# devitocodes/seigen

Hardware: AMD Instinct MI355X
Metric: M DoF-updates/sec, 3D elastic P=4 (higher is better)
Workload: dtype f64

## Files before the change

### seigen_amd/csrc/api.cpp

```cpp
#include <limits>
#include <string>

#include "handle.hpp"
#include "source_tables.hpp"
#include "sponge_tables.hpp"

static int init_element(const sg_config* cfg, sg_handle* h) {
  if (cfg->dim < 1 || cfg->dim > 3) return fail(h, SG_ERR_ARG, "dim must be 1, 2 or 3");
  if (cfg->degree < 1 || cfg->degree > 4) return fail(h, SG_ERR_ARG, "degree must be 1..4");
  for (int a = 0; a < cfg->dim; ++a) {
    if (cfg->n[a] < 1) return fail(h, SG_ERR_ARG, "n[axis] must be >= 1");
    if (!(cfg->h[a] > 0.0)) return fail(h, SG_ERR_ARG, "h[axis] must be > 0");
  }
  h->cfg = *cfg;
  for (int a = cfg->dim; a < 3; ++a) {
    h->cfg.n[a] = 1;
    h->cfg.h[a] = 1.0;
    h->cfg.origin[a] = 0.0;
    h->cfg.cube0[a] = 0;
  }
  int ndev = 0;
  if (hipGetDeviceCount(&ndev) != hipSuccess || ndev <= 0)
    return fail(h, SG_ERR_DEVICE, "no HIP device available (libseigen_hip has no CPU fallback)");
  if (cfg->device < 0 || cfg->device >= ndev) return fail(h, SG_ERR_ARG, "device ordinal out of range");
// ... 97 lines not shown
      Dt = hexm_table(cfg->degree, Dt.data(), Dt.data() + (size_t)(cfg->degree + 1) * (cfg->degree + 1), h->md);
      break;
    }
    case Family::Lane: {
      if (hex) break;
      double fact = 1.0;
      for (int i = 2; i <= d - 1; ++i) fact *= i;
      const double cfold = 1.0 / (2.0 * fact);
      for (int r = 0; r < d; ++r)
        for (int a = 0; a < nd; ++a)
          for (int b = 0; b < nd; ++b) {
            double v = re.D[((size_t)r * nd + a) * nd + b];
            for (int bf = 0; bf < nf; ++bf) {
              if (re.fnode[(size_t)0 * nf + bf] == b) v -= cfold * re.L[((size_t)0 * nd + a) * nf + bf];
              if (re.fnode[(size_t)(r + 1) * nf + bf] == b) v += cfold * re.L[((size_t)(r + 1) * nd + a) * nf + bf];
            }
            Dt[((size_t)r * nd + a) * nd + b] = v;
          }
      Lt = re.L;
      break;
    }
    case Family::Mfma: {
      if (h->f32) set_frags(fr, mfma32_frags_F(re), mfma32_frags_G(re), mfma32_frags_L(re));
      else set_frags(fr, mfma_frags_F(re), mfma_frags_G(re), mfma_frags_L(re));
      const char* gq = std::getenv("SEIGEN_HIP_GQ");
      if (!h->f32 && cfg->degree >= 3 && (gq ? std::atoi(gq) != 0 : cfg->degree >= SG_GQ_FROM_DEGREE)) {
        try {
          fr[3] = mfma_frags_Q(re);
          fr[4] = mfma_frags_P(re);
        } catch (const std::exception& e) {
          return fail(h, SG_ERR_ARG, e.what());
        }
      }
      break;
    }
    case Family::Tile2d: {
      h->t2c = tile2d_const(h->md);
      if (h->f32) set_frags(fr, tile2d_frags32_V(re, -1.0), tile2d_frags32_V(re, 1.0), tile2d_frags32_L(re));
      else set_frags(fr, tile2d_frags_V(re, -1.0), tile2d_frags_V(re, 1.0), tile2d_frags_L(re));
      break;
    }
  }
  HIPCHECK(h, h->Dt.upload(Dt.data(), Dt.size()));
  HIPCHECK(h, h->Lt.upload(Lt.data(), Lt.size()));
  HIPCHECK(h, h->md_dev.upload(&h->md, 1));
  if (h->family == Family::Mfma) {
    const MfmaConst mk = mfma_const(h->md);
    HIPCHECK(h, h->mk_dev.upload(&mk, 1));
    std::vector<int32_t> ft, tab;
    mfma_trace_offsets(h->md, 9, ft);
    HIPCHECK(h, h->ftab_dev.upload(ft.data(), ft.size()));
    if ((h->md.ncube_pad / 16) * 6 * 16 >= ((int64_t)1 << 31))
      return fail(h, SG_ERR_ARG, "block too large for the MFMA path's neighbour table");
    build_nbr_table(h->md, tab);
    HIPCHECK(h, h->nbr_tab.upload(tab.data(), tab.size()));
  }
  return SG_OK;
}

static int init_fields(sg_handle* h, const Frags& fr) {
  const int d = h->cfg.dim, nd = h->re.nd;
  for (int f = 0; f < 4; ++f) {
    size_t comps = field_is_stress(f) ? (size_t)d * d : (size_t)d;
    h->field_len[f] = (size_t)h->ncells * nd * comps;
    h->field_alloc[f] = (size_t)h->md.ncube_pad * h->ncls * nd * comps;
    const size_t n = h->f32 ? (h->field_alloc[f] + 1) / 2 : h->field_alloc[f];
// ... 2 lines not shown
  }
  DevBuf<double>* frag[5] = {&h->fragF, &h->fragG, &h->fragL, &h->fragQ, &h->fragP};
  for (int i = 0; i < 5; ++i)
    if (!fr[i].empty()) HIPCHECK(h, frag[i]->upload(fr[i].data(), fr[i].size()));
  if (family_interleaved(h->family)) {
    const char* sym_env = std::getenv("SEIGEN_HIP_SYM");
    h->sym = !(sym_env && std::strcmp(sym_env, "0") == 0);
    const int zero = 0;
    HIPCHECK(h, h->sym_flag.upload(&zero, 1));
  }
  if (std::getenv("SEIGEN_HIP_STAMPS")) {
    const std::vector<unsigned long long> zeros(32, 0);
    HIPCHECK(h, h->dbg.upload(zeros.data(), zeros.size()));
  }
  return SG_OK;
}

static int blocks_per_cu(const sg_handle* h) {
  const int P = h->cfg.degree;
  return h->family == Family::Mfma ? mfma_blocks_per_cu(P, h->f32) : (h->family == Family::Hexm ? hexm_blocks_per_cu(P) : 2);
}

static int init_launch(sg_handle* h) {
  const sg_config* cfg = &h->cfg;
  hipDeviceProp_t prop;
  HIPCHECK(h, hipGetDeviceProperties(&prop, cfg->device));
  h->ncu = prop.multiProcessorCount;
  const int slots = blocks_per_cu(h) * prop.multiProcessorCount;
  h->grid_full = slots / 8 * 8;
  h->grid_blocks = (cfg->nbr_mask != 0 ? slots - slots / 16 : slots) / 8 * 8;
  if (const char* gb = std::getenv("SEIGEN_HIP_GRID_BLOCKS")) h->grid_blocks = std::max(8, std::atoi(gb) / 8 * 8);
  if (cfg->nbr_mask == 0) h->grid_full = h->grid_blocks;
  h->order_chunk = 0;
  if (h->family == Family::Mfma) {
    const int64_t per_layer = ((int64_t)cfg->n[0] * cfg->n[1] + 15) / 16 * 6;
    if (cfg->n[2] >= 16) h->order_chunk = (int)std::max<int64_t>(6, (per_layer + 7) / 8);
  }
  if (const char* oc = std::getenv("SEIGEN_HIP_ORDER_CHUNK")) h->order_chunk = std::max(0, std::atoi(oc));
  h->no_whole = std::getenv("SEIGEN_HIP_NO_WHOLE") != nullptr;
  h->tile_grid = 0;
  h->tile_grid_sponge = 2008;
  if (const char* tg = std::getenv("SEIGEN_HIP_TILE_GRID")) h->tile_grid = h->tile_grid_sponge = std::max(8, std::atoi(tg) / 8 * 8);
  const char* ge = std::getenv("SEIGEN_HIP_GRAPH");
  const int64_t dofs = h->ncells * (int64_t)h->re.nd * (cfg->dim + cfg->dim * cfg->dim);
  h->graph_ok = ge ? (std::strcmp(ge, "0") != 0) : (dofs <= (int64_t)1 << 23);
  const char* ov = std::getenv("SEIGEN_HIP_OVERLAP");
  h->overlap = cfg->nbr_mask != 0 && !(ov && std::strcmp(ov, "0") == 0);
  int prio_lo = 0, prio_hi = 0;
  HIPCHECK(h, hipDeviceGetStreamPriorityRange(&prio_lo, &prio_hi));
  if (cfg->stream) {
    h->stream = (hipStream_t)cfg->stream;
  } else {
    HIPCHECK(h, hipStreamCreateWithPriority(&h->stream, hipStreamNonBlocking, h->overlap ? prio_hi : 0));
    h->own_stream = true;
  }
  if (h->overlap) {
    HIPCHECK(h, hipStreamCreateWithPriority(&h->stream2, hipStreamNonBlocking, prio_lo));
    HIPCHECK(h, hipEventCreateWithFlags(&h->ev_stage, hipEventDisableTiming));
    HIPCHECK(h, hipEventCreateWithFlags(&h->ev_second, hipEventDisableTiming));
  }
  HIPCHECK(h, hipEventCreate(&h->ev0));
  HIPCHECK(h, hipEventCreate(&h->ev1));
  HIPCHECK(h, hipDeviceSynchronize());
  return SG_OK;
}

// ... 457 lines not shown
```

### seigen_amd/csrc/handle.hpp

```cpp
#pragma once
#include <hip/hip_runtime.h>

#include <cmath>
#include <algorithm>
#include <cstdio>
#include <cstdlib>
#include <cstring>
#include <string>
#include <thread>
#include <vector>

#include "../../include/seigen_hip.h"
#include "hostlogic.hpp"
#include "kernels.hpp"
#include "mesh_tables.hpp"
#include "mfma_tables.hpp"
#include "refelem.hpp"

using namespace sg;

struct sg_comm_state;

template <typename T>
struct DevBuf {
// ... 95 lines not shown
  const double* read(int f) const { return buf_[f].get(); }
  double* write(int f) {
    ver_.written(f);
    return buf_[f].get();
  }
  void replayed() { ver_.replayed(); }
  const FieldVersions& versions() const { return ver_; }
  hipError_t alloc(int f, size_t n) { return buf_[f].alloc(n); }

 private:
  DevBuf<double> buf_[4];
  FieldVersions ver_;
};

struct sg_handle {
  sg_config cfg;
  sg_comm_state* comm = nullptr;
  RefElem re;
  MeshDev md;
  DevBuf<MeshDev> md_dev;
  DevBuf<double> Dt, Lt;
  Fields field;
  size_t field_len[4] = {0, 0, 0, 0};
  size_t field_alloc[4] = {0, 0, 0, 0};
  Family family = Family::Generic;
  int f32 = 0;
  bool sym = false;
  DevBuf<int> sym_flag;
  DevBuf<int32_t> region_items[5];
  int32_t region_nitems[5] = {-1, -1, -1, -1, -1};
  bool region_whole[5] = {false, false, false, false, false};
  DevBuf<double> fragF, fragG, fragL;
  DevBuf<double> fragQ, fragP;
  DevBuf<double> staging;
  double* pin[2] = {nullptr, nullptr};
  DevBuf<double> dstage[2];
  hipEvent_t xfer_ev[2] = {nullptr, nullptr};
  DevBuf<unsigned long long> dbg;
  size_t staging_len = 0;
  int64_t ncells = 0;
  int ncls = 0;
  bool params_set = false;
  double rho = 1.0, dt = 0.0, lam0 = 0.0, mu0 = 0.0;
  int per_cell = 0;
  DevBuf<double> lam_d, mu_d;
  DevBuf<double> rho2_d;
  int rho_physical = 0;
  SpongeTables sponge;
  SourceTables src;
  int64_t src_step = 0;
  DevBuf<int64_t> src_ctr_d;
  bool graph_src = false;
  ReceiverTables rec;
  bool graph_rec = false;
  MonitorTables mon;
  MeasureScratch msr;
  bool graph_mon = false;
  const double* ghost[4][6] = {};
  hipStream_t stream = nullptr;
  bool own_stream = false;
  bool overlap = false;
  hipStream_t stream2 = nullptr;
  hipEvent_t ev_stage = nullptr, ev_second = nullptr;
  bool second_pending = false;
  DevBuf<int32_t> nbr_tab;
  DevBuf<MfmaConst> mk_dev;
// ... 71 lines not shown
```

### seigen_amd/csrc/kernels.hpp

```cpp
#pragma once
#include <cstdint>
#include <string>
#include <type_traits>
#include <vector>

#include "../../include/seigen_hip.h"
#include "mesh_tables.hpp"

namespace sg {

constexpr int SG_MAX_BOXES = 7;

template <int DIM, int P, int TP = 0>
struct ElemDims {
  static constexpr int ND = TP ? (DIM == 3 ? (P + 1) * (P + 1) * (P + 1) : (P + 1) * (P + 1))
                               : (DIM == 1) ? (P + 1) : (DIM == 2) ? (P + 1) * (P + 2) / 2 : (P + 1) * (P + 2) * (P + 3) / 6;
  static constexpr int NF = (DIM == 1) ? 1 : (DIM == 2) ? (P + 1) : (TP ? (P + 1) * (P + 1) : (P + 1) * (P + 2) / 2);
  static constexpr int NFACES = TP ? 2 * DIM : DIM + 1;
  static constexpr int NCLS = TP ? 1 : (DIM == 1) ? 1 : (DIM == 2) ? 2 : 6;
};

constexpr int MK_KSF = 4;
constexpr int MK_KS = 9;
#ifndef SG_GQ_FROM_DEGREE
// ... 50 lines not shown
  const double* Lt;
  const MeshDev* md;
  const MfmaConst* mk;
  const int32_t* ftab;
  const int32_t* nbr_tab;
  int32_t all_active;
  int32_t tensor;
  const double* fragV;
  const double* fragL;
  const double* fragQ;
  unsigned long long* dbg;
  const int32_t* sponge_slot;
  const double* sponge_B;
  const double* sponge_sigma;
  const void* sponge_pre;
  const double* lam;
  const double* mu;
  double lam0, mu0;
  double c_self, c_aux, c_new;
  const double* rho2;
  int32_t mode;
  int32_t per_cell;
  int32_t box_o[3], box_n[3];
  int32_t nbox;
  int32_t boxes_o[SG_MAX_BOXES][3], boxes_n[SG_MAX_BOXES][3];
  int32_t spread;
  const int32_t* item_list;
  int32_t nlist;
  int32_t sym;
  int32_t grid_blocks;
  int32_t f32;
  int32_t order_chunk;
  int32_t nitems;
  void* reserved_;
  const int32_t* src_slot;
  const int32_t* src_idx;
  const double* src_vals;
  double src_scale;
  double src_coef;
  SrcStep src_step;
  int32_t src_bump;
};

std::string kernel_name_of(const void* host_fn);

template <int V0, int... Vs, typename F>
auto sg_pick(int v, F&& f) {
  decltype(f(std::integral_constant<int, V0>())) r{};
  auto take = [&](auto c) { return v == c.value && ((r = f(c)), true); };
  (void)(take(std::integral_constant<int, V0>()) || ... || take(std::integral_constant<int, Vs>()));
  return r;
}
inline int any_ghost(const StageArgs& a, int nsides) {
  int g = 0;
  for (int sd = 0; sd < nsides; ++sd) g |= a.ghost[sd] != nullptr;
  return g;
}

const void* stage_kernel_generic(int kind, int dim, int P, const StageArgs& a);
int launch_stage(const void* kernel, int dim, int P, const StageArgs& a, void* stream);

int mfma_blocks_per_cu(int P, int f32);
const void* stage_kernel_mfma(int kind, int P, const StageArgs& a);
int launch_stage_mfma(const void* kernel, const StageArgs& a, void* stream);

const void* stage_kernel_lane(int kind, int dim, int P, const StageArgs& a);
int launch_stage_lane(const void* kernel, const StageArgs& a, long nitems, void* stream);
int hexm_blocks_per_cu(int P);
std::vector<double> hexm_table(int P, const double* D1, const double* lift1, const MeshDev& md_host);
const void* stage_kernel_hexm(int kind, int P, const StageArgs& a);
int launch_stage_hexm(const void* kernel, int P, const StageArgs& a, long nitems, void* stream);

struct T2Class {
  double Jinv[2][2], cn[4][2];
  int32_t nb_axis[4], nb_dir[4], nb_cls[4];
  int32_t slot_ord[4];
  uint32_t tfw[4][2];
  uint32_t tgw[4][2];
};
struct T2Const {
  int32_t n0, n1, ncube, ngroups;
  int32_t has_nbr[4];
  int32_t halo_per_cube;
  int32_t gpr;
  double inv_n0;
  uint32_t tpw[4][2];
  T2Class cls[2];
};
T2Const tile2d_const(const MeshDev& md_host);
const void* stage_kernel_tile2d(int kind, int P, const StageArgs& a);
int launch_stage_tile2d(const void* kernel, int resident, const StageArgs& a, const T2Const& c, long nitems, void* stream);

int launch_layout(const MeshDev& md_host, int ncomp, int dir, void* field, double* staging, int64_t cell0,
                  int64_t ncells, int sym, int* flag, int f32, void* stream);
int launch_mirror(const MeshDev& md_host, void* field, int f32, void* stream);
// ... 59 lines not shown
```

### seigen_amd/csrc/kernels_mfma.hip

```cpp
#include <hip/hip_runtime.h>

#include "kernels.hpp"

namespace sg {

template <typename R>
struct RT;
template <>
struct RT<double> {
  typedef double v4 __attribute__((ext_vector_type(4)));
  static constexpr bool SMALL = true;
  static __device__ __forceinline__ v4 big(double a, double b, v4 c) { return __builtin_amdgcn_mfma_f64_16x16x4f64(a, b, c, 0, 0, 0); }
  static __device__ __forceinline__ double small(double a, double b, double c) { return __builtin_amdgcn_mfma_f64_4x4x4f64(a, b, c, 0, 0, 0); }
};
template <>
struct RT<float> {
  typedef float v4 __attribute__((ext_vector_type(4)));
  static constexpr bool SMALL = false;
  static __device__ __forceinline__ v4 big(float a, float b, v4 c) { return __builtin_amdgcn_mfma_f32_16x16x4f32(a, b, c, 0, 0, 0); }
  static __device__ __forceinline__ float small(float, float, float c) { return c; }
};

template <typename R, int P>
constexpr int mfma_resident_blocks() {
  return sizeof(R) == 4 ? 3 : (P == 1 ? 4 : (P == 2 ? 3 : 2));
}

template <int P, typename R>
struct MG {
  static constexpr int ND = ElemDims<3, P>::ND;
  static constexpr int NF = ElemDims<3, P>::NF;
  static constexpr int KS = (ND + 3) / 4;
  static constexpr int KSF = (NF + 3) / 4;
  static constexpr int MTF = RT<R>::SMALL ? ND / 16 : (ND + 15) / 16;
  static constexpr int NSM = RT<R>::SMALL ? (ND % 16 + 3) / 4 : 0;
  static constexpr int MTT = MTF + NSM;
  static constexpr int MTFA = MTF > 0 ? MTF : 1;
  static constexpr int NSMA = NSM > 0 ? NSM : 1;
  static constexpr int S4 = (ND + 3) / 4;
  static constexpr int NFRAG_F = MTT * 3 * KS;
  static constexpr int NFRAG_G = 3 * MTT * KS;
  static constexpr int NFRAG_L = 4 * MTT * KSF;
  static constexpr int RK = (P >= 2) ? ElemDims<3, (P >= 2 ? P - 1 : 1)>::ND : 1;
  static constexpr int QLT = RK / 16;
  static constexpr int QST = (RK % 16 + 3) / 4;
  static constexpr int KR = (RK + 3) / 4;
  static constexpr int NFRAG_Q = (QLT + QST) * KS;
  static constexpr int NFRAG_P = 3 * MTT * KR;
};

#define LD_STREAM(p) __builtin_nontemporal_load(p)
#define ST_STREAM(p, v) __builtin_nontemporal_store((v), (p))
#define SG_PRIO(p) __builtin_amdgcn_s_setprio(p)
constexpr int SG_PRIO_F0 = 0x120, SG_PRIO_F1 = 0x320, SG_PRIO_F2 = 0x320, SG_PRIO_G0 = 0x120, SG_PRIO_G1 = 0x120;
#define SG_PRIO_VOL ((PRIO3 >> 8) & 3)
#define SG_PRIO_LIFT ((PRIO3 >> 4) & 3)
#define SG_PRIO_EPI (PRIO3 & 3)
#define MFMA64(a, b, c) RT<R>::big((a), (b), (c))
#define MFMA4(a, b, c) RT<R>::small((a), (b), (c))

#ifdef SG_STAMPS
#define STAMP(t)                                                                   \
  do {                                                                             \
    __builtin_amdgcn_sched_barrier(0);                                             \
    asm volatile("s_memtime %0\n\ts_waitcnt lgkmcnt(0)" : "=s"(t)::"memory");       \
    __builtin_amdgcn_sched_barrier(0);                                             \
  } while (0)
#define STAMP_DECL unsigned long long st0 = 0, st1 = 0, st2 = 0, st3 = 0, st4 = 0, sta = 0, stb = 0, sacc[4] = {0, 0, 0, 0}, ssub[3] = {0, 0, 0}, sitems = 0
#define STAMP_ACC                                                                  \
  do {                                                                             \
    sacc[0] += st1 - st0;                                                          \
    sacc[1] += st2 - st1;                                                          \
    sacc[2] += st3 - st2;                                                          \
    sacc[3] += st4 - st3;                                                          \
    if (sta) { ssub[0] += sta - st2; ssub[1] += stb - sta; ssub[2] += st3 - stb; } \
    sitems += 1;                                                                   \
  } while (0)
#define STAMP_FLUSH                                                                \
  do {                                                                             \
    if (A.dbg && lane == 0) {                                                      \
      for (int z = 0; z < 4; ++z) atomicAdd(&A.dbg[z], sacc[z]);                   \
// ... 162 lines not shown
    r.xcd = xcd;
    r.lo = slot * wpb + wave;
    r.hi = mine > 0 ? mine * chunk : 0;
    return r;
  }
  const long ipx = (nitems + 7) / 8;
  r.lo = xcd * ipx + slot * wpb + wave;
  r.hi = (xcd + 1) * ipx < nitems ? (xcd + 1) * ipx : nitems;
  return r;
}
__device__ __forceinline__ long item_of(const ItemRange& r, long it) {
  if (r.chunk == 0) return it;
  const long c = it / r.chunk;
  const long item = (c * 8 + r.xcd) * r.chunk + (it - c * r.chunk);
  return item < r.nitems ? item : -1;
}

template <int N, typename R, int NT = 256>
__device__ __forceinline__ void copy_to_lds(R* dst, const R* __restrict__ src) {
  constexpr int PER = (N + NT - 1) / NT;
  R v[PER];
#pragma unroll
  for (int j = 0; j < PER; ++j) {
    const int i = threadIdx.x + j * NT;
    v[j] = (i < N) ? src[i] : R(0);
  }
#pragma unroll
  for (int j = 0; j < PER; ++j) {
    const int i = threadIdx.x + j * NT;
    if (i < N) dst[i] = v[j];
  }
}

template <int NV, int NL, typename R, int NT = 256>
__device__ __forceinline__ void load_tables(R* sAV, R* sAL, const StageArgs& A) {
  copy_to_lds<NV * 64, R, NT>(sAV, reinterpret_cast<const R*>(A.fragV));
  copy_to_lds<NL * 64, R, NT>(sAL, reinterpret_cast<const R*>(A.fragL));
  __syncthreads();
}

template <int NV, int NL, typename R>
__device__ __forceinline__ void load_tables(R* sAV, R* sAL, MeshDev* sMd, const StageArgs& A) {
  const int* src = reinterpret_cast<const int*>(A.md);
  int* dst = reinterpret_cast<int*>(sMd);
  constexpr int NI = (int)(sizeof(MeshDev) / sizeof(int)), PERI = (NI + 255) / 256;
  int w[PERI];
#pragma unroll
  for (int j = 0; j < PERI; ++j) {
    const int i = threadIdx.x + j * 256;
    w[j] = (i < NI) ? src[i] : 0;
  }
  copy_to_lds<NV * 64>(sAV, reinterpret_cast<const R*>(A.fragV));
  copy_to_lds<NL * 64>(sAL, reinterpret_cast<const R*>(A.fragL));
#pragma unroll
  for (int j = 0; j < PERI; ++j) {
    const int i = threadIdx.x + j * 256;
    if (i < NI) dst[i] = w[j];
  }
  __syncthreads();
}


template <typename R>
__device__ __forceinline__ R ndot(R c0, R c1, R c2, R t0, R t1, R t2) {
  R r = c0 * t0;
  r = __builtin_fma(c1, t1, r);
  r = __builtin_fma(c2, t2, r);
  return r;
}
template <>
__device__ __forceinline__ float ndot<float>(float c0, float c1, float c2, float t0, float t1, float t2) {
  float r = c0 * t0;
  r = __builtin_fmaf(c1, t1, r);
  r = __builtin_fmaf(c2, t2, r);
  return r;
}


template <typename R, int P, int MODE, int SYM, int FACT>
__global__ __launch_bounds__(256, (mfma_resident_blocks<R, P>())) void mfma_stage_G(StageArgs A) {
  using M = MG<P, R>;
  typedef typename RT<R>::v4 d4;
  constexpr int PRIO3 = MODE ? SG_PRIO_G1 : SG_PRIO_G0;
  constexpr int ND = M::ND, NF = M::NF, KS = M::KS, KSF = M::KSF, MTF = M::MTF, NSM = M::NSM, MTT = M::MTT, S4 = M::S4;
  constexpr int PF = sizeof(R) == 4 ? 6 : 4;
  constexpr int QLT = M::QLT, QST = M::QST, KR = M::KR;
  __shared__ R sAV[(FACT ? M::NFRAG_P : M::NFRAG_G) * 64];
  __shared__ R sQ[FACT ? M::NFRAG_Q * 64 : 1];
  __shared__ R sAL[M::NFRAG_L * 64];
  __shared__ MeshDev sMd;
  if constexpr (FACT) copy_to_lds<M::NFRAG_Q * 64>(sQ, reinterpret_cast<const R*>(A.fragQ));
  load_tables<(FACT ? M::NFRAG_P : M::NFRAG_G), M::NFRAG_L>(sAV, sAL, &sMd, A);

  const int lane = threadIdx.x & 63;
  const int wave = __builtin_amdgcn_readfirstlane(threadIdx.x >> 6);
  const int q = lane >> 4, w = lane & 15;
  typedef __attribute__((address_space(4))) const MeshDev cMeshDev;
  const cMeshDev* md = (const cMeshDev*)(unsigned long long)A.md;
  const R* __restrict__ in = reinterpret_cast<const R*>(A.in);
  R* __restrict__ out = reinterpret_cast<R*>(A.out);
  const R c_self = (R)A.c_self, c_new = (R)A.c_new;
  const long ngroups = sMd.ncube_pad >> 4;
  const ItemRange ir = item_range(A.item_list ? (long)A.nlist : ngroups * 6, wave, A.spread, A.order_chunk);

  STAMP_DECL;
  for (long it = ir.lo; it < ir.hi; it += ir.step) {
    STAMP(st0);
    const long iti = item_of(ir, it);
    if (iti < 0) continue;
    const long item = A.item_list ? (long)A.item_list[iti] : iti;
    const long g = item / 6;
    const int k = (int)(item - g * 6);
    const LaneGeo L = A.all_active ? lane_geo_all(sMd.ncube, g, w) : lane_geo(sMd, A, g, w);
    const nbr4 nbe = load_nbr4(A, item, w);
    if (!__any(L.active)) continue;
    const R* own = in + ((g * 6 + k) * (long)ND) * 3 * 16 + w;
    int qo = q * 3 * 16;
    asm volatile("" : "+v"(qo));
    const R* ownq = own + qo;
    const R* ownl = (4 * (KS - 1) + q < ND) ? ownq + (KS - 1) * 4 * 3 * 16 : own;
    auto brow = [&](int ks) { return (ks == KS - 1) ? ownl : ownq + ks * 4 * 3 * 16; };
    int lo = lane;
    asm volatile("" : "+v"(lo));

    R Jm[3][3], cnf[4][3];
#pragma unroll
    for (int r = 0; r < 3; ++r)
#pragma unroll
      for (int j = 0; j < 3; ++j) Jm[r][j] = (R)(-md->Jinv[k][r][j]);
#pragma unroll
    for (int f = 0; f < 4; ++f)
#pragma unroll
      for (int j = 0; j < 3; ++j) cnf[f][j] = (R)md->cn[k][f][j];

    R Sd[3][S4], So[3][S4];
#pragma unroll
    for (int i = 0; i < 3; ++i)
#pragma unroll
      for (int m = 0; m < S4; ++m) Sd[i][m] = So[i][m] = R(0);

    constexpr int NB = 2;
    constexpr int NBO = FACT ? NB : 1;
    R nx[NB][KSF][3], nxo[NBO][KSF][3];
    auto request = [&](int f, R (&dst)[KSF][3], R (&dso)[KSF][3]) {
      const NbrRef<R> NR = nbr_from_entry<ND, NF, 3>(A, nbe[f], 2 * sMd.nb_axis[k][f] + (sMd.nb_dir[k][f] > 0 ? 1 : 0), own);
#pragma unroll
      for (int ks = 0; ks < KSF; ++ks) {
        const int bb = (4 * ks + q < NF) ? 4 * ks + q : 0;
        const int on = sMd.fnode[f][bb];
        const int nn = NR.ghost ? sMd.nb_fnode[k][f][bb] : (NR.physical ? on : sMd.nb_node[k][f][bb]);
#pragma unroll
        for (int i = 0; i < 3; ++i) {
          dst[ks][i] = NR.p[(nn * 3 + i) * NR.cstride];
          if constexpr (FACT) dso[ks][i] = own[(on * 3 + i) * 16];
        }
      }
    };
    SG_PRIO(SG_PRIO_VOL);
    STAMP(st1);
    auto fold_dir = [&](int r, const d4 (&acc)[M::MTFA][3], const R (&accs)[M::NSMA][3]) {
#pragma unroll
      for (int kk = 0; kk < 3; ++kk) {
        const R c = Jm[r][kk];
        if (uniform_nonzero(c)) {
#pragma unroll
          for (int i = 0; i < 3; ++i) {
#pragma unroll
            for (int t = 0; t < MTF; ++t)
#pragma unroll
              for (int reg = 0; reg < 4; ++reg) {
                if (4 * t + reg >= S4) continue;
                if (i == kk)
                  Sd[i][4 * t + reg] += c * acc[t][i][reg];
                else
                  So[i + kk - 1][4 * t + reg] += c * acc[t][i][reg];
              }
#pragma unroll
            for (int t = 0; t < NSM; ++t) {
              if (i == kk)
                Sd[i][4 * MTF + t] += c * accs[t][i];
              else
                So[i + kk - 1][4 * MTF + t] += c * accs[t][i];
            }
          }
        }
      }
#pragma unroll
      for (int m = 0; m < S4; ++m)
#pragma unroll
        for (int i = 0; i < 3; ++i) asm volatile("" : "+v"(Sd[i][m]), "+v"(So[i][m]));
    };
    auto tiles_step = [&](int nks, int r, int ks, const R (&b)[3], d4 (&acc)[M::MTFA][3], R (&accs)[M::NSMA][3]) {
#pragma unroll
      for (int t = 0; t < MTT; ++t) {
        const R a = sAV[((r * MTT + t) * nks + ks) * 64 + lo];
#pragma unroll
        for (int i = 0; i < 3; ++i) {
          if (t < MTF)
            acc[t < MTF ? t : 0][i] = MFMA64(a, b[i], acc[t < MTF ? t : 0][i]);
          else
            accs[t < MTF ? 0 : t - MTF][i] = MFMA4(a, b[i], accs[t < MTF ? 0 : t - MTF][i]);
        }
      }
    };
    auto clear_acc = [&](d4 (&acc)[M::MTFA][3], R (&accs)[M::NSMA][3]) {
#pragma unroll
      for (int i = 0; i < 3; ++i) {
#pragma unroll
        for (int t = 0; t < MTF; ++t) acc[t][i] = d4{0, 0, 0, 0};
#pragma unroll
        for (int t = 0; t < NSM; ++t) accs[t][i] = R(0);
      }
    };
    if constexpr (!FACT) {
      constexpr int NS = 3 * KS;
      R bq[PF][3];
#pragma unroll
      for (int s = 0; s < PF; ++s)
#pragma unroll
        for (int i = 0; i < 3; ++i) bq[s][i] = brow(s % KS)[i * 16];
#pragma unroll
      for (int r = 0; r < 3; ++r) {
        d4 acc[M::MTFA][3];
        R accs[M::NSMA][3];
        clear_acc(acc, accs);
#pragma unroll
        for (int ks = 0; ks < KS; ++ks) {
          const int s = r * KS + ks;
// ... 2 lines not shown
          for (int i = 0; i < 3; ++i) b[i] = bq[s % PF][i];
          if (s + PF < NS) {
#pragma unroll
            for (int i = 0; i < 3; ++i) bq[s % PF][i] = brow((s + PF) % KS)[i * 16];
          }
          tiles_step(KS, r, ks, b, acc, accs);
        }
        fold_dir(r, acc, accs);
      }
    } else {
      d4 yl[QLT > 0 ? QLT : 1][3];
      R ys[QST > 0 ? QST : 1][3];
#pragma unroll
      for (int i = 0; i < 3; ++i) {
#pragma unroll
        for (int t = 0; t < QLT; ++t) yl[t][i] = d4{0, 0, 0, 0};
#pragma unroll
        for (int t = 0; t < QST; ++t) ys[t][i] = R(0);
      }
      R bq[PF][3];
#pragma unroll
      for (int s = 0; s < PF && s < KS; ++s)
#pragma unroll
        for (int i = 0; i < 3; ++i) bq[s][i] = brow(s)[i * 16];
#pragma unroll
      for (int ks = 0; ks < KS; ++ks) {
        R b[3];
#pragma unroll
        for (int i = 0; i < 3; ++i) b[i] = bq[ks % PF][i];
        if (ks + PF < KS) {
#pragma unroll
          for (int i = 0; i < 3; ++i) bq[ks % PF][i] = brow(ks + PF)[i * 16];
        }
#pragma unroll
        for (int t = 0; t < QLT + QST; ++t) {
          const R a = sQ[(t * KS + ks) * 64 + lo];
#pragma unroll
          for (int i = 0; i < 3; ++i) {
            if (t < QLT)
              yl[t < QLT ? t : 0][i] = MFMA64(a, b[i], yl[t < QLT ? t : 0][i]);
            else
              ys[t < QLT ? 0 : t - QLT][i] = MFMA4(a, b[i], ys[t < QLT ? 0 : t - QLT][i]);
          }
        }
      }
#pragma unroll
      for (int r = 0; r < 3; ++r) {
        d4 acc[M::MTFA][3];
        R accs[M::NSMA][3];
        clear_acc(acc, accs);
#pragma unroll
        for (int ks = 0; ks < KR; ++ks) {
          R b[3];
#pragma unroll
          for (int i = 0; i < 3; ++i) b[i] = (ks < 4 * QLT) ? yl[(ks / 4) < QLT ? ks / 4 : 0][i][ks % 4] : ys[(ks - 4 * QLT) >= 0 && (ks - 4 * QLT) < QST ? ks - 4 * QLT : 0][i];
          tiles_step(KR, r, ks, b, acc, accs);
        }
        fold_dir(r, acc, accs);
      }
    }

    STAMP(st2);
    {
#pragma unroll
      for (int f0 = 0; f0 < NB - 1; ++f0) request(f0, nx[f0], nxo[f0 % NBO]);
      SG_PRIO(SG_PRIO_LIFT);
#pragma unroll
      for (int f = 0; f < 4; ++f) {
        R(&flf)[KSF][3] = nx[f % NB];
        if constexpr (FACT) {
#pragma unroll
          for (int ks = 0; ks < KSF; ++ks)
#pragma unroll
            for (int i = 0; i < 3; ++i) flf[ks][i] += nxo[f % NBO][ks][i];
        }
#pragma unroll
        for (int t = 0; t < MTT; ++t) {
          if (t == 0 && f + NB - 1 < 4) request(f + NB - 1, nx[(f + NB - 1) % NB], nxo[(f + NB - 1) % NBO]);
          auto fold = [&](int m0, int nm, const R (&v)[3][4]) {
#pragma unroll
            for (int kk = 0; kk < 3; ++kk) {
              const R c = cnf[f][kk];
              if (uniform_nonzero(c)) {
#pragma unroll
                for (int i = 0; i < 3; ++i)
#pragma unroll
                  for (int j = 0; j < 4; ++j)
                    if (j < nm && m0 + j < S4) {
                      if (i == kk)
                        Sd[i][m0 + j] += c * v[i][j];
                      else
                        So[i + kk - 1][m0 + j] += c * v[i][j];
                    }
              }
            }
#pragma unroll
            for (int j = 0; j < 4; ++j)
              if (j < nm && m0 + j < S4) {
#pragma unroll
                for (int i = 0; i < 3; ++i) asm volatile("" : "+v"(Sd[i][m0 + j]), "+v"(So[i][m0 + j]));
              }
          };
          if (t < MTF) {
            d4 tmp[3];
#pragma unroll
            for (int i = 0; i < 3; ++i) tmp[i] = d4{0, 0, 0, 0};
#pragma unroll
            for (int ks = 0; ks < KSF; ++ks) {
              const R a = sAL[((f * MTT + t) * KSF + ks) * 64 + lo];
#pragma unroll
              for (int i = 0; i < 3; ++i) tmp[i] = MFMA64(a, flf[ks][i], tmp[i]);
            }
            {
              R v[3][4];
#pragma unroll
              for (int i = 0; i < 3; ++i)
#pragma unroll
                for (int reg = 0; reg < 4; ++reg) v[i][reg] = tmp[i][reg];
              fold(4 * t, 4, v);
            }
          } else {
            R tmp[3] = {R(0), R(0), R(0)};
#pragma unroll
            for (int ks = 0; ks < KSF; ++ks) {
              const R a = sAL[((f * MTT + t) * KSF + ks) * 64 + lo];
#pragma unroll
              for (int i = 0; i < 3; ++i) tmp[i] = MFMA4(a, flf[ks][i], tmp[i]);
            }
            {
              const R v[3][4] = {{tmp[0], 0, 0, 0}, {tmp[1], 0, 0, 0}, {tmp[2], 0, 0, 0}};
              fold(4 * MTF + (t - MTF), 1, v);
            }
          }
        }
      }
    }

    SG_PRIO(SG_PRIO_EPI);
    STAMP(st3);
    {
      const long e = (L.valid ? L.c : 0) * 6 + k;
      const R lam = (R)(A.per_cell ? A.lam[e] : A.lam0);
      const R mu = (R)(A.per_cell ? A.mu[e] : A.mu0);
      const long obase = ((g * 6 + k) * (long)ND) * 9 * 16 + w;
      int qo9 = q * 9 * 16;
      asm volatile("" : "+v"(qo9));
      const long ob_q = obase + qo9;
      const long ob_l = (4 * (S4 - 1) + q < ND) ? ob_q + (long)(S4 - 1) * 4 * 9 * 16 : obase;
      auto orow = [&](int m) { return (m == S4 - 1) ? ob_l : ob_q + (long)m * 4 * 9 * 16; };
      if constexpr (SYM || MODE == 0) {
        constexpr int NL = SYM ? 6 : 9;
        constexpr int PDE = 4;
        R po[PDE][6];
        auto line = [](int c) { return SYM ? (c < 3 ? c : (c < 5 ? c + 1 : 8)) : c; };
        auto fetch_old = [&](int m) {
          const long o1 = orow(m);
#pragma unroll
          for (int c = 0; c < 6; ++c) po[m % PDE][c] = LD_STREAM(&out[o1 + line(c) * 16]);
// ... 37 lines not shown
              ST_STREAM(&out[o + 3 * 16], So[0][m]);
              ST_STREAM(&out[o + 6 * 16], So[1][m]);
              ST_STREAM(&out[o + 7 * 16], So[2][m]);
            }
          }
        }
        (void)NL;
      } else {
#pragma unroll
        for (int m = 0; m < S4; ++m) {
          const int a = 4 * m + q;
          const long o = orow(m);
          const R tr = lam * (Sd[0][m] + Sd[1][m] + Sd[2][m]);
          R s[9];
          s[0] = R(2) * mu * Sd[0][m] + tr;
          s[4] = R(2) * mu * Sd[1][m] + tr;
          s[8] = R(2) * mu * Sd[2][m] + tr;
          s[1] = s[3] = mu * So[0][m];
          s[2] = s[6] = mu * So[1][m];
          s[5] = s[7] = mu * So[2][m];
#pragma unroll
          for (int ij = 0; ij < 9; ++ij) s[ij] = c_self * out[o + ij * 16] + c_new * s[ij];
          if (L.active && a < ND) {
#pragma unroll
            for (int ij = 0; ij < 9; ++ij) out[o + ij * 16] = s[ij];
          }
        }
      }
    }
    STAMP(st4);
    STAMP_ACC;
  }
  STAMP_FLUSH;
}

template <typename R, int P, int MODE, int SYM, int GHOST>
__global__ __launch_bounds__(256, (mfma_resident_blocks<R, P>())) void mfma_stage_F(StageArgs A) {
  using M = MG<P, R>;
  typedef typename RT<R>::v4 d4;
  constexpr int PRIO3 = MODE == 1 ? SG_PRIO_F1 : (MODE == 2 ? SG_PRIO_F2 : SG_PRIO_F0);
  constexpr int ND = M::ND, NF = M::NF, KS = M::KS, KSF = M::KSF, MTF = M::MTF, NSM = M::NSM, MTT = M::MTT;
  __shared__ R sAV[M::NFRAG_F * 64];
  __shared__ R sAL[M::NFRAG_L * 64];
  __shared__ nbr4 sFt[3 * 6 * 4 * 4];
  {
    const nbr4* src = reinterpret_cast<const nbr4*>(A.ftab);
    for (int i = threadIdx.x; i < 3 * 6 * 4 * 4; i += 256) sFt[i] = src[i];
  }
  load_tables<M::NFRAG_F, M::NFRAG_L>(sAV, sAL, A);
  const cMfmaConst& mk = *(const cMfmaConst*)(unsigned long long)A.mk;

  const int lane = threadIdx.x & 63;
  const int wave = __builtin_amdgcn_readfirstlane(threadIdx.x >> 6);
  const int q = lane >> 4, w = lane & 15;
  typedef __attribute__((address_space(4))) const MeshDev cMeshDev;
  const cMeshDev* md = (const cMeshDev*)(unsigned long long)A.md;
  const R* __restrict__ in = reinterpret_cast<const R*>(A.in);
  const R* __restrict__ aux = reinterpret_cast<const R*>(A.aux);
  R* __restrict__ out = reinterpret_cast<R*>(A.out);
  const R c_self = (R)A.c_self, c_aux = (R)A.c_aux, c_new = (R)A.c_new;
  const long ngroups = mk.ncube_pad >> 4;
  const ItemRange ir = item_range(A.item_list ? (long)A.nlist : ngroups * 6, wave, A.spread, A.order_chunk);

  STAMP_DECL;
  for (long it = ir.lo; it < ir.hi; it += ir.step) {
    STAMP(st0);
// ... 390 lines not shown
    default: return -1;
  }
  return (int)hipGetLastError();
}

int mfma_blocks_per_cu(int P, int f32) {
  if (f32) return mfma_resident_blocks<float, 4>();
  return P == 1 ? mfma_resident_blocks<double, 1>() : (P == 2 ? mfma_resident_blocks<double, 2>() : mfma_resident_blocks<double, 4>());
}

const void* stage_kernel_mfma(int kind, int P, const StageArgs& a) {
  return sg_pick<0, 1>(a.f32 != 0, [&](auto f32) {
    using R = std::conditional_t<decltype(f32)::value, float, double>;
    return sg_pick<1, 2, 3, 4>(P, [&](auto p) {
      constexpr int PP = decltype(p)::value, HAS_FACT = sizeof(R) == 8 && PP >= 3;
      return sg_pick<0, 1>(a.sym != 0, [&](auto sym) {
        constexpr int SYM = decltype(sym)::value;
        if (kind == 0)
          return sg_pick<0, 1, 2>(a.mode == 0 || a.mode == 2 ? a.mode : 1, [&](auto mode) {
            return sg_pick<0, 1>(any_ghost(a, 6), [&](auto ghost) {
              return (const void*)&mfma_stage_F<R, PP, decltype(mode)::value, SYM, decltype(ghost)::value>;
            });
          });
        return sg_pick<0, 1>(a.mode != 0, [&](auto mode) {
          return sg_pick<0, HAS_FACT>(HAS_FACT && a.fragQ != nullptr, [&](auto fact) {
            return (const void*)&mfma_stage_G<R, PP, decltype(mode)::value, SYM, decltype(fact)::value>;
          });
        });
      });
    });
  });
}

int launch_stage_mfma(const void* kernel, const StageArgs& a, void* stream) {
  unsigned nblk = (unsigned)(a.grid_blocks > 0 ? a.grid_blocks : 512);
  if (a.nitems > 0 && !a.spread) {
    const unsigned need = (((unsigned)a.nitems + 3u) / 4u + 7u) / 8u * 8u;
    nblk = need < nblk ? need : nblk;
  }
  void* args[] = {const_cast<StageArgs*>(&a)};
  (void)hipLaunchKernel(kernel, dim3(nblk), dim3(256), args, 0, (hipStream_t)stream);
  return (int)hipGetLastError();
}

}
```

### seigen_amd/csrc/stages.cpp

```cpp
#include "handle.hpp"


struct LaunchCtx {
  hipStream_t stream;
  bool capture_src = false;
  bool capture_rec = false;
  bool capture_mon = false;
};

struct SourceNow {
  SourceSlice at;
  const double* values;
  SrcStep stepper;
};
static SourceSlice source_at(const sg_handle* h, bool capture) {
  const SourceTables& src = h->src;
  return source_slice({src.nnz, src.nsteps, src.is_static, src.weights.empty() ? nullptr : src.weights.data(), h->cfg.dim}, h->src_step,
                      capture);
}
static SourceNow source_now(const sg_handle* h, const LaunchCtx& ctx) {
  SourceNow sn;
  sn.at = source_at(h, ctx.capture_src);
  sn.values = h->src.values.get() + sn.at.offset;
  std::memset(&sn.stepper, 0, sizeof(sn.stepper));
// ... 2 lines not shown
    sn.stepper.nsteps = sn.at.nsteps;
    sn.stepper.stride = sn.at.stride;
    sn.stepper.weights = sn.at.use_weights ? h->src.weights_d.get() : nullptr;
    sn.stepper.is_static = sn.at.is_static ? 1 : 0;
  }
  return sn;
}

static int stage_args(sg_handle* h, const LaunchCtx& ctx, StageArgs& a, const StageOp& op, int region) {
  const int kind = op.kind;
  if (kind != 0 && kind != 1) return fail(h, SG_ERR_ARG, "unknown stage");
  std::memset(&a, 0, sizeof(a));
  a.in = h->field.read(op.in);
  a.aux = op.aux >= 0 ? h->field.read(op.aux) : nullptr;
  a.uabs = h->field.read(op.uabs);
  for (int s = 0; s < 6; ++s) {
    a.ghost[s] = h->ghost[op.in][s];
    if (h->md.has_nbr[s] && !a.ghost[s])
      return fail(h, SG_ERR_STATE, "stage needs a halo buffer that was not attached (sg_halo_attach)");
  }
  a.Dt = h->Dt.get();
  a.Lt = h->Lt.get();
  a.md = h->md_dev.get();
  a.mk = h->mk_dev.get();
  a.ftab = h->ftab_dev.get();
  a.nbr_tab = h->nbr_tab.get();
  a.all_active = region == SG_REGION_ALL ? 1 : 0;
  a.tensor = h->re.kind == KIND_TENSOR ? 1 : 0;
  a.fragV = (kind == 0) ? h->fragF.get() : h->fragG.get();
  a.fragL = h->fragL.get();
  if (kind == 1 && h->fragQ.get()) {
    a.fragV = h->fragP.get();
    a.fragQ = h->fragQ.get();
  }
  a.sym = h->sym ? 1 : 0;
  a.f32 = h->f32;
  const SpongeTables& sp = h->sponge;
  a.dbg = h->dbg.get() ? h->dbg.get() + 8 * (kind * 2 + (op.mode ? 1 : 0)) : nullptr;
  a.sponge_slot = (kind == 0) ? sp.slot.get() : nullptr;
  a.sponge_B = sp.B.get();
  a.sponge_sigma = (kind == 0) ? sp.sigma.get() : nullptr;
  a.sponge_pre = (kind == 0) ? sp.pre.get() : nullptr;
  a.lam = h->lam_d.get();
  a.mu = h->mu_d.get();
  a.lam0 = h->lam0;
  a.mu0 = h->mu0;
  a.per_cell = h->per_cell;
  a.rho2 = op.density ? h->rho2_d.get() : nullptr;
  a.src_coef = op.src_coef;
  a.mode = op.mode;
  a.c_self = op.c_self;
  a.c_aux = op.c_aux;
  a.c_new = op.c_new;
  if (!h->src.fused) return SG_OK;
  const SourceNow sn = source_now(h, ctx);
  if (kind == 0 && op.in == SG_FIELD_S && op.mode == 0 && ctx.capture_src) {
    a.src_step = sn.stepper;
    a.src_bump = 1;
  }
  if (op.with_source && sn.at.due) {
    a.src_slot = h->src.slot.get();
    a.src_idx = h->src.idx.get();
    a.src_vals = sn.values;
    a.src_scale = sn.at.scale;
    a.src_step = sn.stepper;
  }
// ... 597 lines not shown
```

Measured before the change: 89570.

## Stash Q-pass B rows in LDS and compact fragment tables for P=4 G stage

For the f64 P=4 factored G stage, the kernel moves to 512-thread blocks with dynamic LDS. Small-tile fragment tables are stored compactly, and each wave stashes the Q-pass B rows in LDS so the face-flux pass reads own-cell values from LDS instead of reloading them from global memory. This removes the extra global loads of the own-side face values and shrinks the fragment table footprint. In exchange occupancy drops to one block per CU, the grid is halved, and there is more LDS traffic plus an extra index table lookup.

```diff
diff --git a/seigen_amd/csrc/api.cpp b/seigen_amd/csrc/api.cpp
--- a/seigen_amd/csrc/api.cpp
+++ b/seigen_amd/csrc/api.cpp
@@ -153,6 +153,8 @@
           return fail(h, SG_ERR_ARG, e.what());
         }
       }
+      const char* gs = std::getenv("SEIGEN_HIP_GSTASH");
+      h->gstash = !(gs && std::atoi(gs) == 0);
       break;
     }
     case Family::Tile2d: {
@@ -221,6 +223,7 @@
   if (const char* gb = std::getenv("SEIGEN_HIP_GRID_BLOCKS")) h->grid_blocks = std::max(8, std::atoi(gb) / 8 * 8);
   if (cfg->nbr_mask == 0) h->grid_full = h->grid_blocks;
   h->order_chunk = 0;
+  if (h->family == Family::Mfma && prepare_stage_mfma() != 0) return fail(h, SG_ERR_DEVICE, "the G stage kernels' dynamic LDS was refused");
   if (h->family == Family::Mfma) {
     const int64_t per_layer = ((int64_t)cfg->n[0] * cfg->n[1] + 15) / 16 * 6;
     if (cfg->n[2] >= 16) h->order_chunk = (int)std::max<int64_t>(6, (per_layer + 7) / 8);
diff --git a/seigen_amd/csrc/handle.hpp b/seigen_amd/csrc/handle.hpp
--- a/seigen_amd/csrc/handle.hpp
+++ b/seigen_amd/csrc/handle.hpp
@@ -151,6 +151,7 @@
   bool region_whole[5] = {false, false, false, false, false};
   DevBuf<double> fragF, fragG, fragL;
   DevBuf<double> fragQ, fragP;
+  bool gstash = true;
   DevBuf<double> staging;
   double* pin[2] = {nullptr, nullptr};
   DevBuf<double> dstage[2];
diff --git a/seigen_amd/csrc/kernels.hpp b/seigen_amd/csrc/kernels.hpp
--- a/seigen_amd/csrc/kernels.hpp
+++ b/seigen_amd/csrc/kernels.hpp
@@ -106,7 +106,8 @@
   int32_t f32;
   int32_t order_chunk;
   int32_t nitems;
-  void* reserved_;
+  int32_t gstash;
+  int32_t reserved_;
   const int32_t* src_slot;
   const int32_t* src_idx;
   const double* src_vals;
@@ -135,6 +136,7 @@
 int launch_stage(const void* kernel, int dim, int P, const StageArgs& a, void* stream);
 
 int mfma_blocks_per_cu(int P, int f32);
+int prepare_stage_mfma();
 const void* stage_kernel_mfma(int kind, int P, const StageArgs& a);
 int launch_stage_mfma(const void* kernel, const StageArgs& a, void* stream);
 
diff --git a/seigen_amd/csrc/kernels_mfma.hip b/seigen_amd/csrc/kernels_mfma.hip
--- a/seigen_amd/csrc/kernels_mfma.hip
+++ b/seigen_amd/csrc/kernels_mfma.hip
@@ -47,6 +47,31 @@
   static constexpr int KR = (RK + 3) / 4;
   static constexpr int NFRAG_Q = (QLT + QST) * KS;
   static constexpr int NFRAG_P = 3 * MTT * KR;
+};
+
+template <typename R, int P, int FACT>
+constexpr bool g_stash() {
+  return sizeof(R) == 8 && P == 4 && FACT == 1;
+}
+template <int NOUT, int LT, int ST, int NKS>
+struct CompactTiles {
+  static constexpr int NL = NOUT * LT * NKS * 64, NS = NOUT * ST * NKS * 16, N = NL + NS;
+  static constexpr int at(int o, int t, int ks) {
+    return t < LT ? ((o * LT + t) * NKS + ks) * 64 : NL + ((o * ST + (t - LT)) * NKS + ks) * 16;
+  }
+};
+constexpr int G_STASH_SLOTS = 36;
+constexpr int G_STASH_WAVES = 8;
+template <typename R, int P, int STASH>
+struct GLds {
+  using M = MG<P, R>;
+  static constexpr int STW = 3 * G_STASH_SLOTS * 16;
+  static constexpr int OFF_FO = ((int)sizeof(MeshDev) + 15) / 16 * 16;
+  static constexpr int OFF_AV = OFF_FO + (STASH ? 64 * (int)sizeof(int) : 0);
+  static constexpr int OFF_Q = OFF_AV + (int)sizeof(R) * (STASH ? CompactTiles<3, M::MTF, M::NSM, M::KR>::N : M::NFRAG_P * 64);
+  static constexpr int OFF_AL = OFF_Q + (int)sizeof(R) * (STASH ? CompactTiles<1, M::QLT, M::QST, M::KS>::N : M::NFRAG_Q * 64);
+  static constexpr int OFF_ST = OFF_AL + (int)sizeof(R) * (STASH ? CompactTiles<4, M::MTF, M::NSM, M::KSF>::N : M::NFRAG_L * 64);
+  static constexpr int BYTES = OFF_ST + (STASH ? G_STASH_WAVES * STW * (int)sizeof(R) : 0);
 };
 
 #define LD_STREAM(p) __builtin_nontemporal_load(p)
@@ -275,6 +300,30 @@
   }
 }
 
+template <typename CT, int NOUT, int LT, int ST, int NKS, typename R, int NT>
+__device__ __forceinline__ void copy_compact(R* dst, const R* __restrict__ src) {
+  constexpr int PER = (CT::N + NT - 1) / NT;
+  R v[PER];
+#pragma unroll
+  for (int j = 0; j < PER; ++j) {
+    const int i = threadIdx.x + j * NT;
+    int s = 0;
+    if (i < CT::NL) {
+      const int fr = i >> 6, o = fr / (LT * NKS), rem = fr - o * (LT * NKS);
+      s = (o * (LT + ST) * NKS + rem) * 64 + (i & 63);
+    } else {
+      const int i2 = i - CT::NL, fr = i2 >> 4, c = i2 & 15, o = fr / (ST * NKS), rem = fr - o * (ST * NKS);
+      s = (o * (LT + ST) * NKS + LT * NKS + rem) * 64 + (c & 3) + 16 * (c >> 2);
+    }
+    v[j] = (i < CT::N) ? src[s] : R(0);
+  }
+#pragma unroll
+  for (int j = 0; j < PER; ++j) {
+    const int i = threadIdx.x + j * NT;
+    if (i < CT::N) dst[i] = v[j];
+  }
+}
+
 template <int NV, int NL, typename R, int NT = 256>
 __device__ __forceinline__ void load_tables(R* sAV, R* sAL, const StageArgs& A) {
   copy_to_lds<NV * 64, R, NT>(sAV, reinterpret_cast<const R*>(A.fragV));
@@ -320,20 +369,54 @@
 }
 
 
-template <typename R, int P, int MODE, int SYM, int FACT>
-__global__ __launch_bounds__(256, (mfma_resident_blocks<R, P>())) void mfma_stage_G(StageArgs A) {
+template <typename R, int P, int MODE, int SYM, bool FACT, bool STASH, bool DYN>
+__device__ __forceinline__ void stage_G_body(const StageArgs& A) {
   using M = MG<P, R>;
+  constexpr int NT = STASH ? 512 : 256;
   typedef typename RT<R>::v4 d4;
   constexpr int PRIO3 = MODE ? SG_PRIO_G1 : SG_PRIO_G0;
   constexpr int ND = M::ND, NF = M::NF, KS = M::KS, KSF = M::KSF, MTF = M::MTF, NSM = M::NSM, MTT = M::MTT, S4 = M::S4;
   constexpr int PF = sizeof(R) == 4 ? 6 : 4;
   constexpr int QLT = M::QLT, QST = M::QST, KR = M::KR;
-  __shared__ R sAV[(FACT ? M::NFRAG_P : M::NFRAG_G) * 64];
-  __shared__ R sQ[FACT ? M::NFRAG_Q * 64 : 1];
-  __shared__ R sAL[M::NFRAG_L * 64];
-  __shared__ MeshDev sMd;
-  if constexpr (FACT) copy_to_lds<M::NFRAG_Q * 64>(sQ, reinterpret_cast<const R*>(A.fragQ));
-  load_tables<(FACT ? M::NFRAG_P : M::NFRAG_G), M::NFRAG_L>(sAV, sAL, &sMd, A);
+  using CP = CompactTiles<3, MTF, NSM, KR>;
+  using CQ = CompactTiles<1, QLT, QST, KS>;
+  using CL = CompactTiles<4, MTF, NSM, KSF>;
+  using LY = GLds<R, P, STASH>;
+  constexpr int STW = LY::STW;
+  R *sAV = nullptr, *sQ = nullptr, *sAL = nullptr, *sSt = nullptr;
+  MeshDev* sMdp = nullptr;
+  int* sFo = nullptr;
+  if constexpr (DYN) {
+    extern __shared__ __attribute__((aligned(16))) unsigned char sg_dyn_lds[];
+    sMdp = reinterpret_cast<MeshDev*>(sg_dyn_lds);
+    sFo = reinterpret_cast<int*>(sg_dyn_lds + LY::OFF_FO);
+    sAV = reinterpret_cast<R*>(sg_dyn_lds + LY::OFF_AV);
+    sQ = reinterpret_cast<R*>(sg_dyn_lds + LY::OFF_Q);
+    sAL = reinterpret_cast<R*>(sg_dyn_lds + LY::OFF_AL);
+    sSt = reinterpret_cast<R*>(sg_dyn_lds + LY::OFF_ST);
+  } else {
+    __shared__ R sAV_[(FACT ? M::NFRAG_P : M::NFRAG_G) * 64];
+    __shared__ R sQ_[FACT ? M::NFRAG_Q * 64 : 1];
+    __shared__ R sAL_[M::NFRAG_L * 64];
+    __shared__ MeshDev sMd_;
+    sAV = sAV_, sQ = sQ_, sAL = sAL_, sMdp = &sMd_;
+  }
+  MeshDev& sMd = *sMdp;
+  if constexpr (STASH) {
+    static_assert(ND <= G_STASH_SLOTS && 4 * KS <= G_STASH_SLOTS, "a stash slot per B row of the Q pass");
+    copy_to_lds<(int)(sizeof(MeshDev) / sizeof(int)), int, NT>(reinterpret_cast<int*>(&sMd), reinterpret_cast<const int*>(A.md));
+    copy_compact<CQ, 1, QLT, QST, KS, R, NT>(sQ, reinterpret_cast<const R*>(A.fragQ));
+    copy_compact<CP, 3, MTF, NSM, KR, R, NT>(sAV, reinterpret_cast<const R*>(A.fragV));
+    copy_compact<CL, 4, MTF, NSM, KSF, R, NT>(sAL, reinterpret_cast<const R*>(A.fragL));
+    if (threadIdx.x < 64) {
+      const int f = threadIdx.x >> 4, bq4 = 4 * (threadIdx.x & 3) + ((threadIdx.x >> 2) & 3);
+      sFo[threadIdx.x] = (int)A.md->fnode[f][bq4 < NF ? bq4 : 0] * 16 * (int)sizeof(R);
+    }
+    __syncthreads();
+  } else {
+    if constexpr (FACT) copy_to_lds<M::NFRAG_Q * 64>(sQ, reinterpret_cast<const R*>(A.fragQ));
+    load_tables<(FACT ? M::NFRAG_P : M::NFRAG_G), M::NFRAG_L>(sAV, sAL, &sMd, A);
+  }
 
   const int lane = threadIdx.x & 63;
   const int wave = __builtin_amdgcn_readfirstlane(threadIdx.x >> 6);
@@ -365,6 +448,10 @@
     auto brow = [&](int ks) { return (ks == KS - 1) ? ownl : ownq + ks * 4 * 3 * 16; };
     int lo = lane;
     asm volatile("" : "+v"(lo));
+    const int lo4 = (lo & 3) + ((lo >> 4) << 2);
+    R* const stw = sSt + (STASH ? wave * STW : 0) + lo;
+    const char* const str = reinterpret_cast<const char*>(sSt + (STASH ? wave * STW : 0) + (lo & 15));
+    auto tile = [&](const R* tab, int full, int at, int t, int nlarge) { return STASH ? tab[at + (t < nlarge ? lo : lo4)] : tab[full * 64 + lo]; };
 
     R Jm[3][3], cnf[4][3];
 #pragma unroll
@@ -383,7 +470,7 @@
       for (int m = 0; m < S4; ++m) Sd[i][m] = So[i][m] = R(0);
 
     constexpr int NB = 2;
-    constexpr int NBO = FACT ? NB : 1;
+    constexpr int NBO = (FACT && !STASH) ? NB : 1;
     R nx[NB][KSF][3], nxo[NBO][KSF][3];
     auto request = [&](int f, R (&dst)[KSF][3], R (&dso)[KSF][3]) {
       const NbrRef<R> NR = nbr_from_entry<ND, NF, 3>(A, nbe[f], 2 * sMd.nb_axis[k][f] + (sMd.nb_dir[k][f] > 0 ? 1 : 0), own);
@@ -395,7 +482,7 @@
 #pragma unroll
         for (int i = 0; i < 3; ++i) {
           dst[ks][i] = NR.p[(nn * 3 + i) * NR.cstride];
-          if constexpr (FACT) dso[ks][i] = own[(on * 3 + i) * 16];
+          if constexpr (FACT && !STASH) dso[ks][i] = own[(on * 3 + i) * 16];
         }
       }
     };
@@ -436,7 +523,7 @@
     auto tiles_step = [&](int nks, int r, int ks, const R (&b)[3], d4 (&acc)[M::MTFA][3], R (&accs)[M::NSMA][3]) {
 #pragma unroll
       for (int t = 0; t < MTT; ++t) {
-        const R a = sAV[((r * MTT + t) * nks + ks) * 64 + lo];
+        const R a = tile(sAV, (r * MTT + t) * nks + ks, CP::at(r, t, ks), t, MTF);
 #pragma unroll
         for (int i = 0; i < 3; ++i) {
           if (t < MTF)
@@ -505,9 +592,13 @@
 #pragma unroll
           for (int i = 0; i < 3; ++i) bq[ks % PF][i] = brow(ks + PF)[i * 16];
         }
+        if constexpr (STASH) {
+#pragma unroll
+          for (int i = 0; i < 3; ++i) stw[(i * G_STASH_SLOTS + 4 * ks) * 16] = b[i];
+        }
 #pragma unroll
         for (int t = 0; t < QLT + QST; ++t) {
-          const R a = sQ[(t * KS + ks) * 64 + lo];
+          const R a = tile(sQ, t * KS + ks, CQ::at(0, t, ks), t, QLT);
 #pragma unroll
           for (int i = 0; i < 3; ++i) {
             if (t < QLT)
@@ -541,7 +632,14 @@
 #pragma unroll
       for (int f = 0; f < 4; ++f) {
         R(&flf)[KSF][3] = nx[f % NB];
-        if constexpr (FACT) {
+        if constexpr (STASH) {
+          const nbr4 fo = *reinterpret_cast<const nbr4*>(&sFo[f * 16 + (lo >> 4) * 4]);
+#pragma unroll
+          for (int ks = 0; ks < KSF; ++ks)
+#pragma unroll
+            for (int i = 0; i < 3; ++i)
+              flf[ks][i] += *reinterpret_cast<const R*>(str + fo[ks] + i * G_STASH_SLOTS * 16 * (int)sizeof(R));
+        } else if constexpr (FACT) {
 #pragma unroll
           for (int ks = 0; ks < KSF; ++ks)
 #pragma unroll
@@ -580,7 +678,7 @@
             for (int i = 0; i < 3; ++i) tmp[i] = d4{0, 0, 0, 0};
 #pragma unroll
             for (int ks = 0; ks < KSF; ++ks) {
-              const R a = sAL[((f * MTT + t) * KSF + ks) * 64 + lo];
+              const R a = tile(sAL, (f * MTT + t) * KSF + ks, CL::at(f, t, ks), t, MTF);
 #pragma unroll
               for (int i = 0; i < 3; ++i) tmp[i] = MFMA64(a, flf[ks][i], tmp[i]);
             }
@@ -596,7 +694,7 @@
             R tmp[3] = {R(0), R(0), R(0)};
 #pragma unroll
             for (int ks = 0; ks < KSF; ++ks) {
-              const R a = sAL[((f * MTT + t) * KSF + ks) * 64 + lo];
+              const R a = tile(sAL, (f * MTT + t) * KSF + ks, CL::at(f, t, ks), t, MTF);
 #pragma unroll
               for (int i = 0; i < 3; ++i) tmp[i] = MFMA4(a, flf[ks][i], tmp[i]);
             }
@@ -700,6 +798,18 @@
     STAMP_ACC;
   }
   STAMP_FLUSH;
+}
+
+template <typename R, int P, int MODE, int SYM, int FACT>
+__global__ __launch_bounds__((g_stash<R, P, FACT>() ? 512 : 256), (g_stash<R, P, FACT>() ? 1 : mfma_resident_blocks<R, P>())) void mfma_stage_G(StageArgs A) {
+  if constexpr (g_stash<R, P, FACT>()) {
+    if (blockDim.x == 512)
+      stage_G_body<R, P, MODE, SYM, true, true, true>(A);
+    else
+      stage_G_body<R, P, MODE, SYM, true, false, true>(A);
+  } else {
+    stage_G_body<R, P, MODE, SYM, FACT != 0, false, false>(A);
+  }
 }
 
 template <typename R, int P, int MODE, int SYM, int GHOST>
@@ -1156,14 +1266,41 @@
   });
 }
 
+static_assert(GLds<double, 4, 1>::BYTES == 156640 && GLds<double, 4, 1>::BYTES <= 160 * 1024, "stash form: one block per CU");
+static_assert(GLds<double, 4, 0>::BYTES == 61152 && 2 * GLds<double, 4, 0>::BYTES <= 160 * 1024, "form without a stash: two blocks per CU");
+
+static bool two_form_kernel(const void* kernel) {
+  for (int v = 0; v < 4; ++v) {
+    const void* k = sg_pick<0, 1>(v & 1, [&](auto mode) {
+      return sg_pick<0, 1>(v >> 1, [&](auto sym) { return (const void*)&mfma_stage_G<double, 4, decltype(mode)::value, decltype(sym)::value, 1>; });
+    });
+    if (k == kernel) return true;
+  }
+  return false;
+}
+
+int prepare_stage_mfma() {
+  for (int v = 0; v < 4; ++v) {
+    const void* k = sg_pick<0, 1>(v & 1, [&](auto mode) {
+      return sg_pick<0, 1>(v >> 1, [&](auto sym) { return (const void*)&mfma_stage_G<double, 4, decltype(mode)::value, decltype(sym)::value, 1>; });
+    });
+    if (hipFuncSetAttribute(k, hipFuncAttributeMaxDynamicSharedMemorySize, GLds<double, 4, 1>::BYTES) != hipSuccess) return -1;
+  }
+  return 0;
+}
+
 int launch_stage_mfma(const void* kernel, const StageArgs& a, void* stream) {
+  const bool two = two_form_kernel(kernel), stash = two && a.gstash;
+  const unsigned wpb = stash ? 8u : 4u;
+  const unsigned lds = two ? (unsigned)(stash ? GLds<double, 4, 1>::BYTES : GLds<double, 4, 0>::BYTES) : 0u;
   unsigned nblk = (unsigned)(a.grid_blocks > 0 ? a.grid_blocks : 512);
+  if (stash) nblk = nblk / 16u * 8u > 8u ? nblk / 16u * 8u : 8u;
   if (a.nitems > 0 && !a.spread) {
-    const unsigned need = (((unsigned)a.nitems + 3u) / 4u + 7u) / 8u * 8u;
+    const unsigned need = (((unsigned)a.nitems + wpb - 1u) / wpb + 7u) / 8u * 8u;
     nblk = need < nblk ? need : nblk;
   }
   void* args[] = {const_cast<StageArgs*>(&a)};
-  (void)hipLaunchKernel(kernel, dim3(nblk), dim3(256), args, 0, (hipStream_t)stream);
+  (void)hipLaunchKernel(kernel, dim3(nblk), dim3(wpb * 64u), args, lds, (hipStream_t)stream);
   return (int)hipGetLastError();
 }
 
diff --git a/seigen_amd/csrc/stages.cpp b/seigen_amd/csrc/stages.cpp
--- a/seigen_amd/csrc/stages.cpp
+++ b/seigen_amd/csrc/stages.cpp
@@ -58,6 +58,7 @@
   if (kind == 1 && h->fragQ.get()) {
     a.fragV = h->fragP.get();
     a.fragQ = h->fragQ.get();
+    a.gstash = h->gstash ? 1 : 0;
   }
   a.sym = h->sym ? 1 : 0;
   a.f32 = h->f32;
```

Measured after the change: 91050 (median of 6 runs). 1.02x the previous value.
